# PoseLib/PoseLib

Hardware: AMD Instinct MI355X
Metric: scored RANSAC hypotheses/sec (P3P@5k corrs, 5pt@5k corrs) (higher is better)
Workload: dtype f64; 1 GPU; p3p_5000; correspondences=5000, problems_in_flight_per_gpu=128, distinct_scenes=64

## Files before the change

### poselib_amd/csrc/kernels.hip

```cpp
#include "pl_kernels.h"
#include "pl_global.h"
#include "pl_lm_chain.inc"
#include "pl_device.h"
#include <atomic>
#include "pl_prefilter.h"
#include <cstdlib>
#include "pl_sampler.h"
#include "pl_solver_h4.h"
#include "pl_solver_p3p.h"
#include "pl_solver_p5lp_radial.h"
#include "pl_solver_rel.h"

namespace pl {

typedef const float __attribute__((address_space(4))) *uniform_f32_ptr;
typedef const double __attribute__((address_space(4))) *uniform_f64_ptr;
typedef const uint32_t __attribute__((address_space(4))) *uniform_u32_ptr;
__device__ __forceinline__ uniform_f32_ptr as_uniform(const float *p) { return (uniform_f32_ptr)(uintptr_t)p; }
__device__ __forceinline__ uniform_f64_ptr as_uniform(const double *p) { return (uniform_f64_ptr)(uintptr_t)p; }
__device__ __forceinline__ uniform_u32_ptr as_uniform(const uint32_t *p) { return (uniform_u32_ptr)(uintptr_t)p; }

__device__ __forceinline__ double wave_sum(double v) {
#pragma unroll
    for (int off = 32; off > 0; off >>= 1)
// ... 1084 lines not shown
        }
    };
    __builtin_amdgcn_fence(__ATOMIC_ACQ_REL, "wavefront");
    Batch b0, b1;
    fetch(n0, first, b0);
    if (n1) {
        fetch(n1, first + n0, b1);
        finish(b0);
        finish(b1);
    } else {
        finish(b0);
    }
}

template <int PG>
__device__ __forceinline__ void abs16_tile_bits(const half8_t (&Aop)[kAbs16Dirs], const uint4 (&s_b)[1 + kAbs16Dirs][PG][32], int col, int half,
                                                uint32_t (&out)[16]) {
#pragma unroll
    for (int v = 0; v < 16; ++v)
        out[v] = 0u;
    const float16_t kZero = {0, 0, 0, 0, 0, 0, 0, 0, 0, 0, 0, 0, 0, 0, 0, 0};
    auto products = [&](int g, float16_t &D0, float16_t &D1, float16_t &D2) {
        half8_t Bop[kAbs16Dirs];
#pragma unroll
        for (int d = 0; d < kAbs16Dirs; ++d) {
            const uint4 braw = s_b[half ? 1 + d : 0][g][col];
            __builtin_memcpy(&Bop[d], &braw, 16);
        }
        D0 = __builtin_amdgcn_mfma_f32_32x32x16_f16(Aop[0], Bop[0], kZero, 0, 0, 0);
        D1 = __builtin_amdgcn_mfma_f32_32x32x16_f16(Aop[1], Bop[1], kZero, 0, 0, 0);
        D2 = __builtin_amdgcn_mfma_f32_32x32x16_f16(Aop[2], Bop[2], kZero, 0, 0, 0);
    };
    float16_t D0, D1, D2;
    products(0, D0, D1, D2);
#pragma unroll 16
    for (int g = 1; g < PG; ++g) {
        uint32_t T[16];
#pragma unroll
        for (int v = 0; v < 16; ++v)
            T[v] = __float_as_uint(D0[v]) | __float_as_uint(D1[v]) | __float_as_uint(D2[v]);
        products(g, D0, D1, D2);
#pragma unroll
        for (int v = 0; v < 16; ++v)
            out[v] = __builtin_amdgcn_alignbit(out[v], T[v], 31);
        __builtin_amdgcn_sched_group_barrier(0x002, 16, 0);
        __builtin_amdgcn_sched_group_barrier(0x100, 3, 0);
        __builtin_amdgcn_sched_group_barrier(0x002, 4, 0);
        __builtin_amdgcn_sched_group_barrier(0x008, 1, 0);
        __builtin_amdgcn_sched_group_barrier(0x002, 4, 0);
        __builtin_amdgcn_sched_group_barrier(0x008, 1, 0);
        __builtin_amdgcn_sched_group_barrier(0x002, 4, 0);
        __builtin_amdgcn_sched_group_barrier(0x008, 1, 0);
        __builtin_amdgcn_sched_group_barrier(0x002, 4, 0);
    }
#pragma unroll
    for (int v = 0; v < 16; ++v) {
        const uint32_t sg = __float_as_uint(D0[v]) | __float_as_uint(D1[v]) | __float_as_uint(D2[v]);
        out[v] = __builtin_amdgcn_alignbit(out[v], sg, 31);
    }
}

constexpr int kScoreAll = 0, kScoreLead = 1, kScoreSel = 2, kScoreCount = 3, kScoreCountAll = 4;
template <int PG, int MODE = kScoreAll>
__device__ __forceinline__ void score_mfma_body(const PointSet &pts, const uint4 *__restrict__ shadow16,
                                                const uint4 *__restrict__ points16,
                                                const double *__restrict__ models, const uint32_t *__restrict__ slots,
                                                const uint32_t *__restrict__ num_hyp_ptr, uint32_t hyp_capacity,
                                                double thr2, uint32_t *__restrict__ part_count,
                                                double *__restrict__ part_score, uint32_t slice, uint32_t chunk,
                                                uint32_t nslices, const uint32_t *__restrict__ sel = nullptr,
                                                uint32_t lead = 0) {
    constexpr int kWaves = kMfmaThreads / 64;
    constexpr int NPW = 32 * PG;
    __shared__ double s_pts[5][NPW];
    __shared__ uint16_t s_queue[kWaves][kMfmaQueueCap];
    __shared__ double s_acc_s[kWaves][64];
    __shared__ uint32_t s_acc_c[kWaves][64];
    __shared__ uint32_t s_next_unit;
    __shared__ uint4 s_b[1 + kAbs16Dirs][PG][32];
    const int lane = threadIdx.x & 63;
    const int wave = __builtin_amdgcn_readfirstlane((int)(threadIdx.x >> 6));
    const int col = lane & 31, half = lane >> 5;

    uint32_t validbits = 0;
#pragma unroll
    for (int g = 0; g < PG; ++g)
        validbits |= (chunk * NPW + g * 32 + col < pts.n) ? (1u << (PG - 1 - g)) : 0u;
    const uint4 *const prow = points16 + (size_t)chunk * NPW * 4;
    for (uint32_t j = threadIdx.x; j < (uint32_t)NPW; j += kMfmaThreads) {
        const uint32_t i = chunk * NPW + j;
        const uint32_t ic = i < pts.n ? i : 0u;
#pragma unroll
        for (int d = 0; d < 5; ++d)
            s_pts[d][j] = pts.a[d][ic];
#pragma unroll
        for (int r = 0; r < 1 + kAbs16Dirs; ++r)
            s_b[r][j >> 5][j & 31] = prow[(size_t)j * 4 + r];
    }
    if (threadIdx.x == 0)
        s_next_unit = 0;
    __syncthreads();

    const uint32_t H = MODE == kScoreLead ? min(*as_uniform(num_hyp_ptr), lead) : *as_uniform(num_hyp_ptr);
    uint16_t *const queue = s_queue[wave];
    double *const acc_s = s_acc_s[wave];
    uint32_t *const acc_c = s_acc_c[wave];
    const uint32_t waves_per_chunk = nslices * kWaves;
    auto request_ticket = [&]() -> uint32_t {
        uint32_t t = 0;
        if (lane == 0) {
            const uint32_t k = atomicAdd(&s_next_unit, 1u);
            t = slice * kWaves + (k % kWaves) + (k / kWaves) * waves_per_chunk;
        }
        return t;
    };
    uint32_t ticket = (uint32_t)__builtin_amdgcn_readfirstlane((int)request_ticket());
    uint32_t kb, gn;
    while (unit_of_ticket<32u>(ticket, H, waves_per_chunk, kb, gn)) {
        const uint32_t pending = request_ticket();
        uint32_t unit_pos = 0;
        if constexpr (MODE == kScoreSel)
            unit_pos = sel ? sel[kb + min((uint32_t)lane, gn - 1u)] : kb + min((uint32_t)lane, gn - 1u);
        const uint32_t unit_slots = slots[MODE == kScoreSel ? unit_pos : kb + min((uint32_t)lane, gn - 1u)];
        acc_s[lane] = 0.0;
        acc_c[lane] = 0;
        uint32_t qhead = 0, qtail = 0;

        auto drain_pair = [&](uint32_t n2) {
            mfma_drain<EST_ABS>(queue, qhead, 64u, n2, &s_pts[0][0], NPW, models, unit_slots, thr2, acc_s, acc_c);
            qhead += 64u + n2;
        };
        auto drain = [&](uint32_t n) {
            mfma_drain<EST_ABS>(queue, qhead, n, 0u, &s_pts[0][0], NPW, models, unit_slots, thr2, acc_s, acc_c);
            qhead += n;
        };

        const uint32_t ngroups32 = (gn + 31u) / 32u;
        auto load_a = [&](uint32_t hg, uint4 (&A)[kAbs16Dirs]) {
            const uint4 *row = shadow16 + (size_t)(kb + 32u * hg + (uint32_t)col) * 4;
            if constexpr (MODE == kScoreSel)
                row = shadow16 + (size_t)(uint32_t)__shfl((int)unit_pos, (int)(32u * hg + (uint32_t)col), 64) * 4;
#pragma unroll
            for (int d = 0; d < kAbs16Dirs; ++d)
                A[d] = row[half ? 3 : d];
        };
        uint4 Araw[kAbs16Dirs];
        load_a(0, Araw);
        for (uint32_t hg = 0; hg < ngroups32; ++hg) {
            half8_t Aop[kAbs16Dirs];
#pragma unroll
            for (int d = 0; d < kAbs16Dirs; ++d)
                __builtin_memcpy(&Aop[d], &Araw[d], 16);
            if (hg + 1 < ngroups32)
                load_a(hg + 1, Araw);
            uint32_t out[16];
            abs16_tile_bits<PG>(Aop, s_b, col, half, out);
            const bool partial_group = hg * 32u + 32u > gn;
            auto expand_round = [&](int v, bool check_slot) {
                const uint32_t slot = hg * 32u + 8u * (uint32_t)(v >> 2) + 4u * (uint32_t)half + (uint32_t)(v & 3);
                uint32_t bits = ~out[v] & validbits;
                if (check_slot && slot >= gn)
                    bits = 0u;
                const uint64_t anyb = __builtin_amdgcn_ballot_w64(bits != 0u);
                if (anyb) {
                    const uint32_t cnt = (uint32_t)__popc(bits);
                    if (!__builtin_amdgcn_ballot_w64(cnt > 1u)) {
                        const uint32_t below = __builtin_amdgcn_mbcnt_hi((uint32_t)(anyb >> 32), __builtin_amdgcn_mbcnt_lo((uint32_t)anyb, 0u));
                        if (bits) {
                            const uint32_t g = (uint32_t)(PG - 1 - (31 - __clz((int)bits)));
                            queue[(qtail + below) & (kMfmaQueueCap - 1)] = (uint16_t)((slot << 9) | (g * 32u + (uint32_t)col));
                        }
                        qtail += (uint32_t)__popcll(anyb);
                    } else {
                        const uint32_t incl = wave_scan_u32(cnt);
                        const uint32_t total = (uint32_t)__builtin_amdgcn_readlane((int)incl, 63);
                        uint32_t pos = qtail + incl - cnt;
                        uint32_t rest = bits;
                        while (rest) {
                            const int hi = 31 - __clz((int)rest);
                            rest &= ~(1u << hi);
                            const uint32_t g = (uint32_t)(PG - 1 - hi);
                            queue[pos & (kMfmaQueueCap - 1)] = (uint16_t)((slot << 9) | (g * 32u + (uint32_t)col));
                            ++pos;
                        }
                        qtail += total;
                    }
                    while (qtail - qhead >= 128u)
                        drain_pair(64u);
                }
            };
            if (partial_group) {
#pragma unroll
                for (int v = 0; v < 16; ++v)
                    expand_round(v, true);
            } else {
#pragma unroll
                for (int v = 0; v < 16; ++v)
                    expand_round(v, false);
            }
        }
        if (qtail - qhead > 64u)
            drain_pair(qtail - qhead - 64u);
        else if (qtail != qhead)
            drain(qtail - qhead);
        __builtin_amdgcn_fence(__ATOMIC_ACQ_REL, "wavefront");
        if ((uint32_t)lane < gn) {
            const size_t o = MODE == kScoreSel ? (size_t)chunk * hyp_capacity + unit_pos : (size_t)chunk * hyp_capacity + kb + lane;
            part_score[o] = acc_s[lane];
            part_count[o] = acc_c[lane];
        }
        ticket = (uint32_t)__builtin_amdgcn_readfirstlane((int)pending);
    }
}

template <int PG>
__device__ __forceinline__ void score_count_body(uint32_t n_points, const uint4 *__restrict__ shadow16, const uint4 *__restrict__ points16,
                                                 const uint32_t *__restrict__ num_hyp_ptr, uint32_t hyp_capacity,
                                                 uint32_t *__restrict__ survivors, uint32_t slice, uint32_t chunk, uint32_t nslices,
                                                 uint32_t first) {
    constexpr int kWaves = kMfmaThreads / 64;
    constexpr int NPW = 32 * PG;
    __shared__ uint4 s_b[1 + kAbs16Dirs][PG][32];
    __shared__ uint32_t s_cnt[kWaves][64];
    __shared__ uint32_t s_next_unit;
    const int lane = threadIdx.x & 63;
    const int wave = __builtin_amdgcn_readfirstlane((int)(threadIdx.x >> 6));
    const int col = lane & 31, half = lane >> 5;
    uint32_t validbits = 0;
#pragma unroll
    for (int g = 0; g < PG; ++g)
        validbits |= (chunk * NPW + g * 32 + col < n_points) ? (1u << (PG - 1 - g)) : 0u;
    const uint4 *const prow = points16 + (size_t)chunk * NPW * 4;
    for (uint32_t j = threadIdx.x; j < (uint32_t)NPW; j += kMfmaThreads) {
#pragma unroll
        for (int r = 0; r < 1 + kAbs16Dirs; ++r)
            s_b[r][j >> 5][j & 31] = prow[(size_t)j * 4 + r];
    }
    if (threadIdx.x == 0)
        s_next_unit = 0;
    __syncthreads();

    const uint32_t Hall = *as_uniform(num_hyp_ptr);
    if (Hall <= first)
        return;
    const uint32_t H = Hall - first;
    uint32_t *const cnt = s_cnt[wave];
    const uint32_t waves_per_chunk = nslices * kWaves;
    auto request_ticket = [&]() -> uint32_t {
        uint32_t t = 0;
        if (lane == 0) {
            const uint32_t k = atomicAdd(&s_next_unit, 1u);
            t = slice * kWaves + (k % kWaves) + (k / kWaves) * waves_per_chunk;
        }
        return t;
    };
    uint32_t ticket = (uint32_t)__builtin_amdgcn_readfirstlane((int)request_ticket());
    uint32_t kb, gn;
    while (unit_of_ticket<32u>(ticket, H, waves_per_chunk, kb, gn)) {
        const uint32_t pending = request_ticket();
        const uint32_t ngroups32 = (gn + 31u) / 32u;
        auto load_a = [&](uint32_t hg, uint4 (&A)[kAbs16Dirs]) {
            const uint4 *row = shadow16 + (size_t)min(first + kb + 32u * hg + (uint32_t)col, Hall - 1u) * 4;
#pragma unroll
            for (int d = 0; d < kAbs16Dirs; ++d)
                A[d] = row[half ? 3 : d];
        };
        uint4 Araw[kAbs16Dirs];
        load_a(0, Araw);
        for (uint32_t hg = 0; hg < ngroups32; ++hg) {
            half8_t Aop[kAbs16Dirs];
#pragma unroll
            for (int d = 0; d < kAbs16Dirs; ++d)
                __builtin_memcpy(&Aop[d], &Araw[d], 16);
            if (hg + 1 < ngroups32)
                load_a(hg + 1, Araw);
            uint32_t out[16];
            abs16_tile_bits<PG>(Aop, s_b, col, half, out);
            uint32_t pk[6] = {0u, 0u, 0u, 0u, 0u, 0u};
#pragma unroll
            for (int v = 0; v < 16; ++v)
                pk[v / 3] += (uint32_t)__popc(~out[v] & validbits) << (10 * (v % 3));
#pragma unroll
            for (int j = 0; j < 6; ++j) {
                uint32_t s = pk[j];
                s += dpp_shift_u32<0x111>(s);
                s += dpp_shift_u32<0x112>(s);
                s += dpp_shift_u32<0x114>(s);
                s += dpp_shift_u32<0x118>(s);
                s += dpp_shift_u32<0x142, 0xa>(s);
                pk[j] = s;
            }
            if (col == 31) {
#pragma unroll
                for (int v = 0; v < 16; ++v)
                    cnt[hg * 32u + 8u * (uint32_t)(v >> 2) + 4u * (uint32_t)half + (uint32_t)(v & 3)] = (pk[v / 3] >> (10 * (v % 3))) & 0x3ffu;
            }
        }
        __builtin_amdgcn_fence(__ATOMIC_ACQ_REL, "wavefront");
        if ((uint32_t)lane < gn)
            survivors[(size_t)chunk * hyp_capacity + first + kb + lane] = cnt[lane];
        __builtin_amdgcn_fence(__ATOMIC_ACQ_REL, "wavefront");
        ticket = (uint32_t)__builtin_amdgcn_readfirstlane((int)pending);
    }
}

template <int PG>
__global__ __launch_bounds__(kMfmaThreads) __attribute__((amdgpu_waves_per_eu(4, 8))) void k_score_mfma(PointSet pts, const uint4 *__restrict__ shadow16,
                                                               const uint4 *__restrict__ points16,
                                                               const double *__restrict__ models,
                                                               const uint32_t *__restrict__ slots,
                                                               const uint32_t *__restrict__ num_hyp_ptr,
                                                               uint32_t hyp_capacity, double thr2,
                                                               uint32_t *__restrict__ part_count,
                                                               double *__restrict__ part_score,
                                                               uint32_t *__restrict__ tickets) {
    (void)tickets;
    uint32_t slice, chunk;
    slice_chunk_of_workgroup(gridDim.x, gridDim.y, slice, chunk);
    score_mfma_body<PG>(pts, shadow16, points16, models, slots, num_hyp_ptr, hyp_capacity, thr2, part_count, part_score, slice,
                        chunk, gridDim.x);
}
template <int PG>
__global__ __launch_bounds__(kMfmaThreads) __attribute__((amdgpu_waves_per_eu(4, 8))) void k_score_mfma_g(const GroupArgs *ga) {
    const GroupArgs &g = ga[blockIdx.z];
    uint32_t slice, chunk;
    if (!g.active || !g.use_mfma || !slice_chunk_of_workgroup(g.slices, g.chunks, slice, chunk))
        return;
    const ScoreArgs a = globalised(g.score);
    score_mfma_body<PG>(a.pts, static_cast<const uint4 *>(a.shadow16), static_cast<const uint4 *>(a.points16), a.models, a.slots,
                        a.num_hyp, a.hyp_capacity, a.thr2, a.part_count, a.part_score, slice, chunk, g.slices);
// ... 104 lines not shown
    uint32_t cs = 0;
    for (uint32_t ch = 0; ch < cstar; ++ch)
        cs += a.part_count[(size_t)ch * a.hyp_capacity + p];
    return prune_rule(cs, 0.0, S, N, a.thr2, *pr.st) ? 0u : 1u;
}
__global__ __launch_bounds__(256) void k_prune_label(ScoreArgs a) {
    const PruneArgs &pr = a.prune;
    const uint32_t H = *a.num_hyp, cstar = pr.st->cstar, p = blockIdx.x * 256u + threadIdx.x;
    if (p >= H || p < pr.lead || cstar >= pr.chunks || pr.kept[p] != kKept)
        return;
    const uint32_t N = a.pts.n, S = min(cstar * pr.chunk_points, N);
    uint32_t cs = 0;
    double sum = 0.0;
    for (uint32_t ch = 0; ch < cstar; ++ch) {
        cs += a.part_count[(size_t)ch * a.hyp_capacity + p];
        sum += a.part_score[(size_t)ch * a.hyp_capacity + p];
    }
    if (prune_rule(cs, sum, S, N, a.thr2, *pr.st))
        pr.kept[p] = kPrunedExact;
}
__device__ __forceinline__ void prune_flags_body(const ScoreArgs &a) {
    __shared__ uint32_t wt[16];
    const PruneArgs &pr = a.prune;
    const uint32_t H = *a.num_hyp, cstar = pr.st->cstar;
    if (blockIdx.x * 1024u >= H)
        return;
    const uint32_t p = blockIdx.x * 1024u + threadIdx.x;
    const uint32_t keep = prune_keeps(a, p, H, cstar);
    if (p < H)
        pr.kept[p] = (uint8_t)keep;
    const uint32_t tot = wave_sum_u32(keep);
    if ((threadIdx.x & 63) == 0)
        wt[threadIdx.x >> 6] = tot;
    __syncthreads();
    if (threadIdx.x == 0) {
        uint32_t t = 0;
        for (int w = 0; w < 16; ++w)
            t += wt[w];
        pr.blk_kept[blockIdx.x] = t;
    }
}
__device__ __forceinline__ void prune_list_body(const ScoreArgs &a) {
    __shared__ uint32_t wt[16], wb[16];
    const PruneArgs &pr = a.prune;
    const uint32_t H = *a.num_hyp;
    if (blockIdx.x * 1024u >= H)
        return;
    const int lane = threadIdx.x & 63, wave = threadIdx.x >> 6;
    uint32_t before = 0;
    for (uint32_t j = threadIdx.x; j < blockIdx.x; j += 1024u)
        before += pr.blk_kept[j];
    before = wave_sum_u32(before);
    const uint32_t p = blockIdx.x * 1024u + threadIdx.x;
    const uint32_t keep = p < H ? (uint32_t)pr.kept[p] : 0u;
    const uint32_t inc = wave_scan_u32(keep);
    if (lane == 63)
        wt[wave] = inc;
    if (lane == 0)
        wb[wave] = before;
    __syncthreads();
    uint32_t at = inc - keep;
    for (int w = 0; w < 16; ++w)
        at += wb[w] + (w < wave ? wt[w] : 0u);
    if (keep)
        pr.sel[at] = p;
    if (p == H - 1u)
        pr.st->sel_len = at + keep;
}
__global__ __launch_bounds__(1024) void k_prune_flags(ScoreArgs a) { prune_flags_body(a); }
__global__ __launch_bounds__(1024) void k_prune_list(ScoreArgs a) { prune_list_body(a); }
__global__ __launch_bounds__(1024) void k_prune_flags_g(const GroupArgs *ga) {
    const GroupArgs &g = ga[blockIdx.z];
    if (!g.active || !g.use_mfma || !g.score.prune.st)
        return;
    prune_flags_body(globalised(g.score));
}
__global__ __launch_bounds__(1024) void k_prune_list_g(const GroupArgs *ga) {
    const GroupArgs &g = ga[blockIdx.z];
    if (!g.active || !g.use_mfma || !g.score.prune.st)
        return;
    prune_list_body(globalised(g.score));
}

constexpr int kBoundThreads = 256;
template <int P, bool RESID>
__device__ __forceinline__ void score_bound_body(const ScoreArgs &a, uint32_t slice, uint32_t chunk, uint32_t nslices) {
    constexpr int kWaves = kBoundThreads / 64;
    constexpr uint32_t NPW = 64u * P;
    const PruneArgs &pr = a.prune;
    if (!pr.st || !pr.bound || *as_uniform(&pr.st->cstar) >= pr.chunks)
        return;
    const uint32_t first = RESID ? 0u : min(*as_uniform(a.num_hyp), pr.lead), len = *as_uniform(&pr.st->sel_len);
    if (len <= first)
        return;
    const int lane = threadIdx.x & 63;
    const int wave = __builtin_amdgcn_readfirstlane((int)(threadIdx.x >> 6));
    const PrefilterArgs pf = a.pf;
    float x[P], y[P], X[P], Y[P], Z[P], fw[P];
    bool valid[P];
    uint64_t vmask[P];
#pragma unroll
    for (int p = 0; p < P; ++p) {
        const uint32_t i = chunk * NPW + (uint32_t)p * 64u + (uint32_t)lane;
        valid[p] = i < a.pts.n;
        vmask[p] = __builtin_amdgcn_ballot_w64(valid[p]);
        const uint32_t ic = valid[p] ? i : 0u;
        const double Xd = a.pts.a[2][ic], Yd = a.pts.a[3][ic], Zd = a.pts.a[4][ic];
        x[p] = (float)a.pts.a[0][ic], y[p] = (float)a.pts.a[1][ic];
        X[p] = (float)Xd, Y[p] = (float)Yd, Z[p] = (float)Zd;
        fw[p] = pf_point_abs(Xd, Yd, Zd, pf.gx);
    }
    const uint32_t nent = len - first;
    for (uint32_t u = slice * kWaves + (uint32_t)wave; u * 64u < nent; u += nslices * kWaves) {
        const uint32_t e = first + u * 64u + (uint32_t)lane;
        const uint32_t pos = pr.sel[min(e, len - 1u)];
        const float4 *sh = reinterpret_cast<const float4 *>(a.models + (size_t)a.slots[pos] * kModelStride + kShadowOff);
        float4 rv[4];
#pragma unroll
        for (int k = 0; k < 4; ++k)
            rv[k] = sh[k];
        const uint32_t n = min(64u, nent - u * 64u);
        uint32_t my_c = 0, my_q = 0;
        for (uint32_t j = 0; j < n; ++j) {
            float r[16];
#pragma unroll
            for (int k = 0; k < 4; ++k) {
                r[4 * k + 0] = __builtin_bit_cast(float, __builtin_amdgcn_readlane(__builtin_bit_cast(int, rv[k].x), (int)j));
                r[4 * k + 1] = __builtin_bit_cast(float, __builtin_amdgcn_readlane(__builtin_bit_cast(int, rv[k].y), (int)j));
                r[4 * k + 2] = __builtin_bit_cast(float, __builtin_amdgcn_readlane(__builtin_bit_cast(int, rv[k].z), (int)j));
                r[4 * k + 3] = __builtin_bit_cast(float, __builtin_amdgcn_readlane(__builtin_bit_cast(int, rv[k].w), (int)j));
            }
            const float gt = pf_abs_bound_slack(r, pf.gx);
            uint32_t c = 0, q = 0;
            if constexpr (RESID) {
#pragma unroll
                for (int p = 0; p < P; ++p) {
                    const float L = pf_abs_r2_lower(r, gt, x[p], y[p], X[p], Y[p], Z[p], fw[p]);
                    c += (uint32_t)__popcll(__builtin_amdgcn_ballot_w64(valid[p] && L < pf.thr2_up));
                    q += valid[p] ? pf_bound_quantum(L, pf.inv_thr2_dn) : 0u;
                }
                q = (uint32_t)__builtin_amdgcn_readlane((int)wave_scan_u32(q), 63);
            } else {
#pragma unroll
                for (int p = 0; p + 1 < P; p += 2) {
                    const v2f Xp = {X[p], X[p + 1]}, Yp = {Y[p], Y[p + 1]}, Zp = {Z[p], Z[p + 1]};
                    const v2f xp = {x[p], x[p + 1]}, yp = {y[p], y[p + 1]}, w = {fw[p], fw[p + 1]};
                    const v2f z0 = pk_fma(bc(r[0]), Xp, pk_fma(bc(r[1]), Yp, pk_fma(bc(r[2]), Zp, bc(r[9]))));
                    const v2f z1 = pk_fma(bc(r[3]), Xp, pk_fma(bc(r[4]), Yp, pk_fma(bc(r[5]), Zp, bc(r[10]))));
                    const v2f z2 = pk_fma(bc(r[6]), Xp, pk_fma(bc(r[7]), Yp, pk_fma(bc(r[8]), Zp, bc(r[11]))));
                    const v2f a0 = pk_fma(-xp, z2, z0);
                    const v2f a1 = pk_fma(-yp, z2, z1);
                    const v2f W = w + bc(gt);
                    const v2f B = pk_fma(bc(pf.thr), z2, W);
#pragma unroll
                    for (int e2 = 0; e2 < 2; ++e2) {
                        const uint64_t out = vmask[p + e2] & (__builtin_amdgcn_ballot_w64(fmaxf(fabsf(a0[e2]), fabsf(a1[e2])) > B[e2]) |
                                                              __builtin_amdgcn_ballot_w64(z2[e2] < -W[e2]));
                        q += (uint32_t)__popcll(out);
                        c += (uint32_t)__popcll(vmask[p + e2] & ~out);
                    }
                }
                if constexpr (P & 1) {
                    constexpr int p = P - 1;
                    const uint64_t out = vmask[p] & __builtin_amdgcn_ballot_w64(pf_abs_outlier(r, gt, pf.thr, x[p], y[p], X[p], Y[p], Z[p], fw[p]));
                    q += (uint32_t)__popcll(out);
                    c += (uint32_t)__popcll(vmask[p] & ~out);
                }
                q <<= 20;
            }
            if ((uint32_t)lane == j)
                my_c = c, my_q = q;
        }
        if ((uint32_t)lane < n) {
            const size_t o = (size_t)chunk * a.hyp_capacity + pos;
            a.part_count[o] = my_c;
            a.part_score[o] = (double)my_q;
        }
    }
}
template <int P, bool RESID> __global__ __launch_bounds__(kBoundThreads) void k_score_bound(ScoreArgs a) {
    uint32_t slice, chunk;
    slice_chunk_of_workgroup(gridDim.x, gridDim.y, slice, chunk);
    score_bound_body<P, RESID>(a, slice, chunk, gridDim.x);
}
template <bool RESID> __global__ __launch_bounds__(kBoundThreads) void k_score_bound_g(const GroupArgs *ga) {
    const GroupArgs &g = ga[blockIdx.z];
    uint32_t slice, chunk;
    const uint32_t ns = pruned_slices<kScoreSel>(g.slices);
    if (!g.active || !g.use_mfma || !g.score.prune.st || !slice_chunk_of_workgroup(ns, g.chunks, slice, chunk))
        return;
    score_bound_body<5, RESID>(globalised(g.score), slice, chunk, ns);
}
__device__ __forceinline__ void prune_bound_body(const ScoreArgs &a, int stage) {
    __shared__ uint32_t wt[16];
    const PruneArgs &pr = a.prune;
    if (!pr.bound || pr.st->cstar >= pr.chunks)
        return;
    const uint32_t first = stage ? 0u : min(*a.num_hyp, pr.lead), len = pr.st->sel_len;
    const uint32_t lead_max = pr.st->lead_max;
    const double beat = pr.st->lead_min * (1.0 + kPruneScoreMargin);
    const int lane = threadIdx.x & 63, wave = threadIdx.x >> 6;
    uint32_t base = 0;
    __syncthreads();
    for (uint32_t t0 = first; t0 < len; t0 += 1024u) {
        const uint32_t e = t0 + threadIdx.x;
        uint32_t keep = 0, p = 0;
        if (e < len) {
            p = pr.sel[e];
            uint32_t c = 0;
            uint64_t q = 0;
#pragma unroll 8
            for (uint32_t ch = 0; ch < pr.chunks; ++ch) {
                c += a.part_count[(size_t)ch * a.hyp_capacity + p];
                q += (uint64_t)a.part_score[(size_t)ch * a.hyp_capacity + p];
            }
            const double qd = (double)q * 9.5367431640625e-07;
            double s_lb = a.thr2 * qd;
            if (fma(a.thr2, qd, -s_lb) < 0.0)
                s_lb = __longlong_as_double(__double_as_longlong(s_lb) - 1);
            keep = (c <= lead_max && s_lb > beat) ? 0u : 1u;
            if (!keep)
                pr.kept[p] = kDropped;
            if (pr.bnd_count)
                pr.bnd_count[p] = c, pr.bnd_score[p] = s_lb;
        }
        const uint32_t inc = wave_scan_u32(keep);
        if (lane == 63)
            wt[wave] = inc;
        __syncthreads();
        uint32_t at = base + inc - keep, tot = 0;
        for (int w = 0; w < 16; ++w) {
            at += w < wave ? wt[w] : 0u;
            tot += wt[w];
        }
        if (keep)
            pr.sel[at] = p;
        base += tot;
        __syncthreads();
    }
    if (threadIdx.x == 0)
        pr.st->sel_len = base;
}
__global__ __launch_bounds__(1024) void k_prune_bound(ScoreArgs a, int stage) { prune_bound_body(a, stage); }
__global__ __launch_bounds__(1024) void k_prune_bound_g(const GroupArgs *ga, int stage) {
    const GroupArgs &g = ga[blockIdx.z];
    if (!g.active || !g.use_mfma || !g.score.prune.st)
        return;
    prune_bound_body(globalised(g.score), stage);
}



template <int EST, int PG>
__device__ __forceinline__ void score_mfma2_body(const PointSet &pts, const uint4 *__restrict__ hypop,
                                                 const double *__restrict__ models, const uint32_t *__restrict__ slots,
                                                 const uint32_t *__restrict__ num_hyp_ptr, uint32_t hyp_capacity,
                                                 double thr2, const PrefilterArgs &pf, uint32_t *__restrict__ part_count,
                                                 double *__restrict__ part_score, uint32_t slice, uint32_t chunk,
                                                 uint32_t nslices) {
    static_assert(EST == EST_REL || EST == EST_FUND, "Sampson scores");
    constexpr int kWaves = kMfmaThreads / 64;
    constexpr int NPW = 32 * PG;
    constexpr int NBR = (EST == EST_REL) ? 6 : 1;
    __shared__ double s_pts[4][NPW];
    __shared__ double s_bear[NBR][(EST == EST_REL) ? NPW : 1];
    __shared__ uint16_t s_queue[kWaves][kMfmaQueueCap];
    __shared__ double s_acc_s[kWaves][64];
    __shared__ uint32_t s_acc_c[kWaves][64];
    __shared__ uint32_t s_next_unit;
    __shared__ uint4 s_bop[PG][3][64];
    const int lane = threadIdx.x & 63;
    const int wave = __builtin_amdgcn_readfirstlane((int)(threadIdx.x >> 6));
    const int col = lane & 31, half = lane >> 5;

    for (uint32_t j = threadIdx.x; j < (uint32_t)NPW; j += kMfmaThreads) {
        const uint32_t i = chunk * NPW + j;
        const uint32_t ic = i < pts.n ? i : 0u;
        const double a0 = pts.a[0][ic], a1 = pts.a[1][ic], b0 = pts.a[2][ic], b1 = pts.a[3][ic];
        s_pts[0][j] = a0, s_pts[1][j] = a1, s_pts[2][j] = b0, s_pts[3][j] = b1;
        if constexpr (EST == EST_REL) {
            const Vec3 u1 = bearing(a0, a1), u2 = bearing(b0, b1);
            s_bear[0][j] = u1.x, s_bear[1][j] = u1.y, s_bear[2][j] = u1.z;
            s_bear[3][j] = u2.x, s_bear[4][j] = u2.y, s_bear[5][j] = u2.z;
        }
    }
    uint32_t validbits = 0;
#pragma unroll
    for (int g = 0; g < PG; ++g)
        validbits |= (chunk * NPW + g * 32 + col < pts.n) ? (1u << (PG - 1 - g)) : 0u;
    for (uint32_t j = threadIdx.x; j < (uint32_t)NPW; j += kMfmaThreads) {
        const uint32_t i = chunk * NPW + j;
        const bool valid = i < pts.n;
        const uint32_t ic = valid ? i : 0u;
        Sampson16Operand o;
        pf16_sampson_point(pts.a[0][ic], pts.a[1][ic], pts.a[2][ic], pts.a[3][ic], valid, pf.t16, o);
#pragma unroll
        for (int b = 0; b < 6; ++b) {
            const uint16_t *h = b < 4 ? o.c + 8 * b : o.s + 8 * (b - 4);
            s_bop[j >> 5][b >> 1][(j & 31) + 32 * (b & 1)] =
                make_uint4((uint32_t)h[0] | ((uint32_t)h[1] << 16), (uint32_t)h[2] | ((uint32_t)h[3] << 16),
                           (uint32_t)h[4] | ((uint32_t)h[5] << 16), (uint32_t)h[6] | ((uint32_t)h[7] << 16));
        }
    }
    if (threadIdx.x == 0)
        s_next_unit = 0;
    __syncthreads();

    const uint32_t H = *as_uniform(num_hyp_ptr);
    const float t16 = pf.t16;
    uint16_t *const queue = s_queue[wave];
    double *const acc_s = s_acc_s[wave];
    uint32_t *const acc_c = s_acc_c[wave];
    const uint32_t waves_per_chunk = nslices * kWaves;
    auto request_ticket = [&]() -> uint32_t {
        uint32_t t = 0;
        if (lane == 0) {
            const uint32_t k = atomicAdd(&s_next_unit, 1u);
            t = slice * kWaves + (k % kWaves) + (k / kWaves) * waves_per_chunk;
        }
        return t;
    };
    uint32_t ticket = (uint32_t)__builtin_amdgcn_readfirstlane((int)request_ticket());
    uint32_t kb, gn;
    while (unit_of_ticket(ticket, H, waves_per_chunk, kb, gn)) {
        const uint32_t pending = request_ticket();
        const uint32_t unit_slots = slots[kb + min((uint32_t)lane, gn - 1u)];
        acc_s[lane] = 0.0;
        acc_c[lane] = 0;
        uint32_t qhead = 0, qtail = 0;

        auto drain = [&](uint32_t n) {
// ... 1934 lines not shown
        k_score_mfma<2 * PP><<<mgrid, mblock, 0, stream>>>(a.pts, static_cast<const uint4 *>(a.shadow16),                \
                                                         static_cast<const uint4 *>(a.points16), a.models, a.slots,    \
                                                         a.num_hyp, a.hyp_capacity, a.thr2, a.part_count, a.part_score, \
                                                         a.tickets);                                                   \
        break;
            switch (P) {
                PL_M_CASE(1)
                PL_M_CASE(2)
                PL_M_CASE(3)
                PL_M_CASE(4)
                PL_M_CASE(5)
            default:
                return hipErrorInvalidValue;
            }
#undef PL_M_CASE
            return hipGetLastError();
        }
    }
    if (streaming) {
        const dim3 qgrid(std::max<uint32_t>(1u, slices * (uint32_t)kScoreThreads / (uint32_t)kQueueThreads), chunks);
        const dim3 qblock(kQueueThreads);
#define PL_Q_CASE(PP)                                                                                                  \
    case PP:                                                                                                           \
        k_score_queue<E, PP><<<qgrid, qblock, 0, stream>>>(a.pts, a.shadow, a.compact64, a.num_hyp, a.hyp_capacity,      \
                                                         a.thr2, pf, a.part_count, a.part_score, a.tickets);           \
        break;
        switch (P) {
            PL_Q_CASE(1)
            PL_Q_CASE(2)
            PL_Q_CASE(3)
            PL_Q_CASE(4)
            PL_Q_CASE(5)
            PL_Q_CASE(6)
        default:
            return hipErrorInvalidValue;
        }
#undef PL_Q_CASE
        return hipGetLastError();
    }
    return hipErrorInvalidValue;
}

hipError_t launch_score_seq(int est, const SeqScoreArgs &a, hipStream_t stream) {
    if (a.cap == 0)
        return hipSuccess;
    const dim3 grid(std::min<uint32_t>(a.cap, 128u)), block(kSeqThreads);
    PL_DISPATCH_EST_0TO5(est, k_score_seq<E><<<grid, block, 0, stream>>>(a));
    return hipGetLastError();
}
int tangent_score_chunk() { return kTangentChunk; }
int radial1d_score_chunk() { return kRadialChunk; }
hipError_t launch_prune_lead(const ScoreArgs &a, hipStream_t stream) {
    k_prune_lead<<<dim3(1), dim3(256), 0, stream>>>(a);
    return hipGetLastError();
}
hipError_t launch_prune_select(const ScoreArgs &a, hipStream_t stream) {
    const uint32_t nb = std::max<uint32_t>(1u, (a.hyp_capacity + 1023u) / 1024u);
    k_prune_flags<<<dim3(nb), dim3(1024), 0, stream>>>(a);
    k_prune_list<<<dim3(nb), dim3(1024), 0, stream>>>(a);
    return hipGetLastError();
}
hipError_t launch_group_prune_lead(const GroupArgs *args, const GroupDims &d, hipStream_t stream) {
    k_prune_lead_g<<<dim3(1, 1, d.G), dim3(256), 0, stream>>>(args);
    return hipGetLastError();
}
hipError_t launch_group_prune_select(const GroupArgs *args, const GroupDims &d, hipStream_t stream) {
    const uint32_t nb = std::max<uint32_t>(1u, (d.max_hcap + 1023u) / 1024u);
    k_prune_flags_g<<<dim3(nb, 1, d.G), dim3(1024), 0, stream>>>(args);
    k_prune_list_g<<<dim3(nb, 1, d.G), dim3(1024), 0, stream>>>(args);
    return hipGetLastError();
}
template <int PG> static hipError_t launch_score_pruned_pg(const ScoreArgs &a, dim3 grid, hipStream_t stream) {
    const dim3 block(kMfmaThreads);
    const dim3 lead_grid(pruned_slices<kScoreLead>(grid.x), grid.y), sel_grid(pruned_slices<kScoreSel>(grid.x), grid.y);
    k_score_mfma_pr<PG, kScoreLead><<<lead_grid, block, 0, stream>>>(a);
    hipError_t e = launch_prune_lead(a, stream);
    if (e != hipSuccess)
        return e;
    k_score_mfma_pr<PG, kScoreCount><<<grid, block, 0, stream>>>(a);
    e = launch_prune_select(a, stream);
    if (e != hipSuccess)
        return e;
    if (a.prune.bound) {
        k_score_bound<PG / 2, false><<<sel_grid, dim3(kBoundThreads), 0, stream>>>(a);
        k_prune_bound<<<dim3(1), dim3(1024), 0, stream>>>(a, 0);
        k_score_bound<PG / 2, true><<<sel_grid, dim3(kBoundThreads), 0, stream>>>(a);
        k_prune_bound<<<dim3(1), dim3(1024), 0, stream>>>(a, 1);
    }
    k_score_mfma_pr<PG, kScoreSel><<<sel_grid, block, 0, stream>>>(a);
    return hipGetLastError();
}
static hipError_t pruned_grid(const ScoreArgs &a, uint32_t slices, dim3 &grid, int &P) {
    uint32_t chunks;
    score_shape(EST_ABS, a.pts.n, true, true, chunks, P);
    if (!a.shadow16 || !a.points16 || !a.prune.st || a.prune.chunks != chunks || a.prune.chunk_points != 64u * (uint32_t)P)
        return hipErrorInvalidValue;
    const uint32_t mslices = std::min<uint32_t>(slices * (uint32_t)kScoreThreads / (uint32_t)kMfmaThreads,
                                                score_slice_limit(EST_ABS, chunks, true));
    grid = dim3(xcd_slices(mslices), chunks);
    return (P == 4 || P == 5) ? hipSuccess : hipErrorInvalidValue;
}
hipError_t launch_score_pruned(const ScoreArgs &a, uint32_t slices, hipStream_t stream) {
    dim3 grid;
    int P;
    const hipError_t e = pruned_grid(a, slices, grid, P);
    if (e != hipSuccess)
        return e;
    return P == 4 ? launch_score_pruned_pg<8>(a, grid, stream) : launch_score_pruned_pg<10>(a, grid, stream);
}
hipError_t launch_score_count(const ScoreArgs &a, uint32_t slices, hipStream_t stream) {
    dim3 grid;
    int P;
    const hipError_t e = pruned_grid(a, slices, grid, P);
    if (e != hipSuccess)
        return e;
    if (P == 4)
        k_score_mfma_pr<8, kScoreCountAll><<<grid, dim3(kMfmaThreads), 0, stream>>>(a);
    else
        k_score_mfma_pr<10, kScoreCountAll><<<grid, dim3(kMfmaThreads), 0, stream>>>(a);
    return hipGetLastError();
}
hipError_t launch_prune_label(const ScoreArgs &a, hipStream_t stream) {
    k_prune_label<<<dim3(std::max<uint32_t>(1u, (a.hyp_capacity + 255u) / 256u)), dim3(256), 0, stream>>>(a);
    return hipGetLastError();
}

hipError_t launch_score(int est, const ScoreArgs &a, uint32_t slices, hipStream_t stream) {
    if (est == EST_RAD1D) {
        if (!a.shadow || !a.compact64)
            return hipErrorInvalidValue;
        const uint32_t chunks = score_chunks(est, a.pts.n, true, false);
        const dim3 qgrid(std::max<uint32_t>(1u, slices * (uint32_t)kScoreThreads / (uint32_t)kQueueThreads), chunks);
        k_score_radial1d<<<qgrid, dim3(kQueueThreads), 0, stream>>>(a.pts, a.shadow, a.compact64, a.num_hyp, a.hyp_capacity, a.thr2, a.pf,
                                                                    a.part_count, a.part_score);
        return hipGetLastError();
    }
    if (est == EST_RELT) {
        if (!a.shadow || !a.compact64)
            return hipErrorInvalidValue;
        const uint32_t chunks = score_chunks(est, a.pts.n, true, false);
        const dim3 qgrid(std::max<uint32_t>(1u, slices * (uint32_t)kScoreThreads / (uint32_t)kQueueThreads), chunks);
        k_score_tangent<<<qgrid, dim3(kQueueThreads), 0, stream>>>(a.pts, a.shadow, a.compact64, a.num_hyp, a.hyp_capacity, a.thr2, a.pf,
                                                                   a.part_count, a.part_score);
        return hipGetLastError();
    }
    PL_DISPATCH_EST(est, return launch_score_est<E>(a, slices, stream));
    return hipSuccess;
}


hipError_t launch_lm(int est, const PointSet &pts, LMTask *tasks, uint32_t num_tasks, hipStream_t stream) {
    const size_t want = sizeof(double) * point_doubles(est) * (size_t)pts.n;
    return launch_lm_tasks(est, tasks, num_tasks, want <= 128 * 1024 ? pts.n : 0u, stream);
}
static std::atomic<int> g_lm_mode{-1};
void set_lm_mode(int mode) { g_lm_mode.store((mode == 1 || mode == 2) ? mode : 0, std::memory_order_release); }
int get_lm_mode() {
    int m = g_lm_mode.load(std::memory_order_acquire);
    if (m < 0) {
        const char *e = std::getenv("POSELIB_AMD_LM_ORDERED");
        m = (e && e[0] == '1') ? 1 : (e && e[0] == '2') ? 2 : 0;
        g_lm_mode.store(m, std::memory_order_release);
    }
    return m;
}
static thread_local int tl_lm_force_ordered = 0;
void set_lm_force_ordered(int on) { tl_lm_force_ordered = on; }
bool lm_sums_ordered(int est) {
    if (tl_lm_force_ordered)
        return true;
// ... 51 lines not shown
        PL_DISPATCH_EST_0123_5(est, k_lm_ordered<E><<<dim3(num_tasks), dim3(kLMThreads), bytes, stream>>>(tasks, (uint32_t)bytes));
    } else {
        PL_DISPATCH_EST_0TO5(est, k_lm<E><<<dim3(num_tasks), dim3(kLMThreads), bytes, stream>>>(tasks, (uint32_t)bytes));
    }
    return hipGetLastError();
}

__global__ void k_task_records(int est, const LMTask *tasks, const double *records_in, double *records_out,
                               uint32_t num_tasks, LMTask *host_tasks) {
    const uint32_t j = blockIdx.x * blockDim.x + threadIdx.x;
    if (j >= num_tasks)
        return;
    if (host_tasks) {
        for (int i = 0; i < kParamDoubles; ++i)
            host_tasks[j].params[i] = tasks[j].params[i];
        host_tasks[j].iterations = tasks[j].iterations;
        host_tasks[j].skipped = tasks[j].skipped;
        host_tasks[j].cost = tasks[j].cost;
        host_tasks[j].initial_cost = tasks[j].initial_cost;
    }
    double *out = records_out + (size_t)j * kModelStride;
    if (tasks[j].skipped) {
        for (int i = 0; i < kModelStride; ++i)
            out[i] = records_in[(size_t)j * kModelStride + i];
    } else {
        record_from_lm_params(est, tasks[j].params, out);
    }
}
__global__ void k_select_record(const double *score_refined, double incumbent_score, const double *rec_refined,
                                const double *rec_incumbent, double *out) {
    const double *src = (*score_refined < incumbent_score) ? rec_refined : rec_incumbent;
    if (threadIdx.x < kModelStride)
        out[threadIdx.x] = src[threadIdx.x];
}
__global__ void k_select_record_g(const SelectArgs *arr) {
    const SelectArgs a = globalised(arr[blockIdx.z]);
    if (!a.out)
        return;
    const double *src = (*a.score_refined < a.incumbent_score) ? a.rec_refined : a.rec_incumbent;
    if (threadIdx.x < kModelStride)
        a.out[threadIdx.x] = src[threadIdx.x];
    if (threadIdx.x == 63 && a.fetch_src)
        *a.fetch_dst = *a.fetch_src;
    if (threadIdx.x == 62 && a.count_out)
        *a.count_out = (*a.score_refined < a.incumbent_score) ? *a.count_refined : a.count_incumbent;
}
hipError_t launch_group_select(const SelectArgs *args, uint32_t G, hipStream_t stream) {
    if (G == 0)
        return hipSuccess;
    k_select_record_g<<<dim3(1, 1, G), dim3(64), 0, stream>>>(args);
    return hipGetLastError();
}
hipError_t launch_group_mask(int est, const MaskArgs *args, uint32_t G, uint32_t max_n, hipStream_t stream) {
    if (G == 0 || max_n == 0)
        return hipSuccess;
    const dim3 grid((max_n + 255) / 256, 1, G), block(256);
    PL_DISPATCH_EST(est, k_mask_g<E><<<grid, block, 0, stream>>>(args));
    return hipGetLastError();
}
hipError_t launch_group_score_seq(int est, const SeqScoreArgs *args, uint32_t G, uint32_t max_cap, hipStream_t stream) {
    if (G == 0 || max_cap == 0)
        return hipSuccess;
    const dim3 grid(std::min<uint32_t>(max_cap, 128u), 1, G), block(kSeqThreads);
    PL_DISPATCH_EST(est, k_score_seq_g<E><<<grid, block, 0, stream>>>(args));
    return hipGetLastError();
}

int group_points_per_lane(int est) { return (est == EST_REL || est == EST_FUND) ? 6 : 5; }

template <int E> static hipError_t launch_group_score_est(const GroupArgs *args, const GroupDims &d, hipStream_t stream) {
    const dim3 grid(std::max<uint32_t>(1u, d.max_slices), std::max<uint32_t>(1u, d.max_chunks), d.G);
    if constexpr (E == EST_ABS) {
        if (d.any_mfma && d.any_prune) {
            const dim3 lead_grid(pruned_slices<kScoreLead>(grid.x), grid.y, grid.z), sel_grid(pruned_slices<kScoreSel>(grid.x), grid.y, grid.z);
            k_score_mfma_pr_g<10, kScoreLead><<<lead_grid, dim3(kMfmaThreads), 0, stream>>>(args);
            hipError_t e = launch_group_prune_lead(args, d, stream);
            if (e != hipSuccess)
                return e;
            k_score_mfma_pr_g<10, kScoreCount><<<grid, dim3(kMfmaThreads), 0, stream>>>(args);
            e = launch_group_prune_select(args, d, stream);
            if (e != hipSuccess)
                return e;
            if (d.any_bound) {
                k_score_bound_g<false><<<sel_grid, dim3(kBoundThreads), 0, stream>>>(args);
                k_prune_bound_g<<<dim3(1, 1, d.G), dim3(1024), 0, stream>>>(args, 0);
                k_score_bound_g<true><<<sel_grid, dim3(kBoundThreads), 0, stream>>>(args);
                k_prune_bound_g<<<dim3(1, 1, d.G), dim3(1024), 0, stream>>>(args, 1);
            }
            k_score_mfma_pr_g<10, kScoreSel><<<sel_grid, dim3(kMfmaThreads), 0, stream>>>(args);
        } else if (d.any_mfma)
            k_score_mfma_g<10><<<grid, dim3(kMfmaThreads), 0, stream>>>(args);
        if (d.any_queue)
            k_score_queue_g<EST_ABS, 5><<<grid, dim3(kQueueThreads), 0, stream>>>(args);
    } else if constexpr (E == EST_HOM) {
        if (d.any_mfma)
            k_score_mfmah_g<10><<<grid, dim3(kMfmaThreads), 0, stream>>>(args);
        if (d.any_queue)
            k_score_queue_g<EST_HOM, 5><<<grid, dim3(kQueueThreads), 0, stream>>>(args);
    } else {
        if (d.any_mfma)
            k_score_mfma2_g<E, 2 * group_mfma2_points_per_lane(E)><<<grid, dim3(kMfmaThreads), 0, stream>>>(args);
        if (d.any_queue)
            k_score_queue_g<E, 6><<<grid, dim3(kQueueThreads), 0, stream>>>(args);
    }
    return hipGetLastError();
}

hipError_t launch_group_score_count(const GroupArgs *args, const GroupDims &d, hipStream_t stream) {
    const dim3 grid(std::max<uint32_t>(1u, d.max_slices), std::max<uint32_t>(1u, d.max_chunks), d.G);
    k_score_mfma_pr_g<10, kScoreCountAll><<<grid, dim3(kMfmaThreads), 0, stream>>>(args);
    return hipGetLastError();
}
hipError_t launch_group_score(int est, const GroupArgs *args, const GroupDims &d, hipStream_t stream) {
    if (d.G == 0)
        return hipSuccess;
    hipError_t e = hipSuccess;
    PL_DISPATCH_EST(est, e = launch_group_score_est<E>(args, d, stream));
    return e;
}

hipError_t launch_group_generate(int est, const GroupArgs *args, uint32_t max_B, uint32_t G, hipStream_t stream) {
    if (G == 0 || max_B == 0)
        return hipSuccess;
    if (est == EST_REL)
        return launch_group_generate_rel(args, max_B, G, stream);
    const dim3 ggrid((max_B + 63) / 64, 1, G), gblock(64);
    PL_DISPATCH_EST(est, k_generate_g<E><<<ggrid, gblock, 0, stream>>>(args));
    return hipGetLastError();
}

hipError_t launch_group_batch(int est, const GroupArgs *args, const GroupDims &d, hipStream_t stream, hipEvent_t ev0,
                              hipEvent_t ev1) {
    if (d.G == 0)
        return hipSuccess;
    hipError_t e = launch_group_positions(sample_size(est), args, d, stream);
    if (e != hipSuccess)
        return e;
    e = launch_group_generate(est, args, d.max_B, d.G, stream);
    if (e != hipSuccess)
        return e;
    e = launch_group_compact(args, d, stream);
    if (e != hipSuccess)
        return e;
    if (ev0 && (e = hipEventRecord(ev0, stream)) != hipSuccess)
        return e;
    e = launch_group_score(est, args, d, stream);
    if (e != hipSuccess)
        return e;
    if (ev1 && (e = hipEventRecord(ev1, stream)) != hipSuccess)
        return e;
    e = launch_group_finalize_records(args, d, stream);
    if (e != hipSuccess)
        return e;
    const uint32_t per_problem = std::max<uint32_t>(16u, std::min<uint32_t>(128u, 4096u / std::max<uint32_t>(1u, d.G)));
    const dim3 sgrid(per_problem, 1, d.G), sblock(kSeqThreads);
    PL_DISPATCH_EST(est, k_score_seq_gb<E><<<sgrid, sblock, 0, stream>>>(args));
    return hipGetLastError();
}

hipError_t launch_task_records(int est, const LMTask *tasks, const double *records_in, double *records_out,
                               uint32_t num_tasks, LMTask *host_tasks, hipStream_t stream) {
    if (num_tasks == 0)
        return hipSuccess;
    k_task_records<<<dim3((num_tasks + 63) / 64), dim3(64), 0, stream>>>(est, tasks, records_in, records_out, num_tasks,
                                                                         host_tasks);
    return hipGetLastError();
}
hipError_t launch_select_record(const double *score_refined, double incumbent_score, const double *rec_refined,
                                const double *rec_incumbent, double *out, hipStream_t stream) {
    k_select_record<<<dim3(1), dim3(64), 0, stream>>>(score_refined, incumbent_score, rec_refined, rec_incumbent, out);
// ... 40 lines not shown
```

Before: 1.268 billion hypotheses/s.

## Fuse two-stage bound scoring into one kernel with in-block reduction and early exit

Merges the cheap bound pass, its prune, the residual bound pass and the second prune into a single k_score_bound kernel. It runs on a fixed grid of 16 workgroups of 512 threads, with waves striding over chunks and per-hypothesis partial counts reduced in shared memory instead of global part_count/part_score arrays. Only hypotheses that survive the first bound are rescored with the residual bound, and the final prune kernel just compacts the list. It also adds an early return in the MFMA score bodies for workgroups with no ticket, done before the shared-memory loads. In exchange, the fixed small grid and non-resident chunk reloads may limit parallelism when there are many hypotheses or chunks.

```diff
diff --git a/poselib_amd/csrc/kernels.hip b/poselib_amd/csrc/kernels.hip
--- a/poselib_amd/csrc/kernels.hip
+++ b/poselib_amd/csrc/kernels.hip
@@ -1190,6 +1190,14 @@
     const int wave = __builtin_amdgcn_readfirstlane((int)(threadIdx.x >> 6));
     const int col = lane & 31, half = lane >> 5;
 
+    const uint32_t H = MODE == kScoreLead ? min(*as_uniform(num_hyp_ptr), lead) : *as_uniform(num_hyp_ptr);
+    const uint32_t waves_per_chunk = nslices * kWaves;
+    {
+        uint32_t kb0, gn0;
+        if (!unit_of_ticket<32u>(slice * kWaves, H, waves_per_chunk, kb0, gn0))
+            return;
+    }
+
     uint32_t validbits = 0;
 #pragma unroll
     for (int g = 0; g < PG; ++g)
@@ -1209,11 +1217,9 @@
         s_next_unit = 0;
     __syncthreads();
 
-    const uint32_t H = MODE == kScoreLead ? min(*as_uniform(num_hyp_ptr), lead) : *as_uniform(num_hyp_ptr);
     uint16_t *const queue = s_queue[wave];
     double *const acc_s = s_acc_s[wave];
     uint32_t *const acc_c = s_acc_c[wave];
-    const uint32_t waves_per_chunk = nslices * kWaves;
     auto request_ticket = [&]() -> uint32_t {
         uint32_t t = 0;
         if (lane == 0) {
@@ -1334,6 +1340,16 @@
     const int lane = threadIdx.x & 63;
     const int wave = __builtin_amdgcn_readfirstlane((int)(threadIdx.x >> 6));
     const int col = lane & 31, half = lane >> 5;
+    const uint32_t Hall = *as_uniform(num_hyp_ptr);
+    if (Hall <= first)
+        return;
+    const uint32_t H = Hall - first;
+    const uint32_t waves_per_chunk = nslices * kWaves;
+    {
+        uint32_t kb0, gn0;
+        if (!unit_of_ticket<32u>(slice * kWaves, H, waves_per_chunk, kb0, gn0))
+            return;
+    }
     uint32_t validbits = 0;
 #pragma unroll
     for (int g = 0; g < PG; ++g)
@@ -1348,12 +1364,7 @@
         s_next_unit = 0;
     __syncthreads();
 
-    const uint32_t Hall = *as_uniform(num_hyp_ptr);
-    if (Hall <= first)
-        return;
-    const uint32_t H = Hall - first;
     uint32_t *const cnt = s_cnt[wave];
-    const uint32_t waves_per_chunk = nslices * kWaves;
     auto request_ticket = [&]() -> uint32_t {
         uint32_t t = 0;
         if (lane == 0) {
@@ -1624,36 +1635,66 @@
     prune_list_body(globalised(g.score));
 }
 
-constexpr int kBoundThreads = 256;
-template <int P, bool RESID>
-__device__ __forceinline__ void score_bound_body(const ScoreArgs &a, uint32_t slice, uint32_t chunk, uint32_t nslices) {
+constexpr int kBoundThreads = 512;
+constexpr uint32_t kBoundGroups = 16;
+template <int P> __device__ __forceinline__ void score_bound_body(const ScoreArgs &a, uint32_t wg, uint32_t nwg) {
     constexpr int kWaves = kBoundThreads / 64;
     constexpr uint32_t NPW = 64u * P;
+    __shared__ uint32_t s_c[kWaves][64];
+    __shared__ uint64_t s_q[kWaves][64];
+    __shared__ uint32_t s_und[64];
+    __shared__ uint32_t s_nund;
     const PruneArgs &pr = a.prune;
     if (!pr.st || !pr.bound || *as_uniform(&pr.st->cstar) >= pr.chunks)
         return;
-    const uint32_t first = RESID ? 0u : min(*as_uniform(a.num_hyp), pr.lead), len = *as_uniform(&pr.st->sel_len);
-    if (len <= first)
+    const uint32_t first = min(*as_uniform(a.num_hyp), pr.lead), len = *as_uniform(&pr.st->sel_len);
+    if (len <= first || (uint64_t)wg * 64u >= len - first)
         return;
     const int lane = threadIdx.x & 63;
     const int wave = __builtin_amdgcn_readfirstlane((int)(threadIdx.x >> 6));
     const PrefilterArgs pf = a.pf;
+    const uint32_t chunks = pr.chunks;
+    const bool resident = chunks <= (uint32_t)kWaves;
     float x[P], y[P], X[P], Y[P], Z[P], fw[P];
     bool valid[P];
     uint64_t vmask[P];
-#pragma unroll
-    for (int p = 0; p < P; ++p) {
-        const uint32_t i = chunk * NPW + (uint32_t)p * 64u + (uint32_t)lane;
-        valid[p] = i < a.pts.n;
-        vmask[p] = __builtin_amdgcn_ballot_w64(valid[p]);
-        const uint32_t ic = valid[p] ? i : 0u;
-        const double Xd = a.pts.a[2][ic], Yd = a.pts.a[3][ic], Zd = a.pts.a[4][ic];
-        x[p] = (float)a.pts.a[0][ic], y[p] = (float)a.pts.a[1][ic];
-        X[p] = (float)Xd, Y[p] = (float)Yd, Z[p] = (float)Zd;
-        fw[p] = pf_point_abs(Xd, Yd, Zd, pf.gx);
-    }
+    auto load_chunk = [&](uint32_t chunk) {
+#pragma unroll
+        for (int p = 0; p < P; ++p) {
+            const uint32_t i = chunk * NPW + (uint32_t)p * 64u + (uint32_t)lane;
+            valid[p] = i < a.pts.n;
+            vmask[p] = __builtin_amdgcn_ballot_w64(valid[p]);
+            const uint32_t ic = valid[p] ? i : 0u;
+            const double Xd = a.pts.a[2][ic], Yd = a.pts.a[3][ic], Zd = a.pts.a[4][ic];
+            x[p] = (float)a.pts.a[0][ic], y[p] = (float)a.pts.a[1][ic];
+            X[p] = (float)Xd, Y[p] = (float)Yd, Z[p] = (float)Zd;
+            fw[p] = pf_point_abs(Xd, Yd, Zd, pf.gx);
+        }
+    };
+    load_chunk(min((uint32_t)wave, chunks - 1u));
+    const uint32_t lead_max = pr.st->lead_max;
+    const double beat = pr.st->lead_min * (1.0 + kPruneScoreMargin);
+    auto decide = [&](uint32_t pos) -> bool {
+        uint32_t c = 0;
+        uint64_t q = 0;
+#pragma unroll
+        for (int w = 0; w < kWaves; ++w) {
+            c += s_c[w][lane];
+            q += s_q[w][lane];
+        }
+        const double qd = (double)q * 9.5367431640625e-07;
+        double s_lb = a.thr2 * qd;
+        if (fma(a.thr2, qd, -s_lb) < 0.0)
+            s_lb = __longlong_as_double(__double_as_longlong(s_lb) - 1);
+        const bool keep = !(c <= lead_max && s_lb > beat);
+        if (!keep)
+            pr.kept[pos] = kDropped;
+        if (pr.bnd_count)
+            pr.bnd_count[pos] = c, pr.bnd_score[pos] = s_lb;
+        return keep;
+    };
     const uint32_t nent = len - first;
-    for (uint32_t u = slice * kWaves + (uint32_t)wave; u * 64u < nent; u += nslices * kWaves) {
+    for (uint32_t u = wg; (uint64_t)u * 64u < nent; u += nwg) {
         const uint32_t e = first + u * 64u + (uint32_t)lane;
         const uint32_t pos = pr.sel[min(e, len - 1u)];
         const float4 *sh = reinterpret_cast<const float4 *>(a.models + (size_t)a.slots[pos] * kModelStride + kShadowOff);
@@ -1662,9 +1703,7 @@
         for (int k = 0; k < 4; ++k)
             rv[k] = sh[k];
         const uint32_t n = min(64u, nent - u * 64u);
-        uint32_t my_c = 0, my_q = 0;
-        for (uint32_t j = 0; j < n; ++j) {
-            float r[16];
+        auto model_of_lane = [&](uint32_t j, float (&r)[16]) {
 #pragma unroll
             for (int k = 0; k < 4; ++k) {
                 r[4 * k + 0] = __builtin_bit_cast(float, __builtin_amdgcn_readlane(__builtin_bit_cast(int, rv[k].x), (int)j));
@@ -1672,17 +1711,17 @@
                 r[4 * k + 2] = __builtin_bit_cast(float, __builtin_amdgcn_readlane(__builtin_bit_cast(int, rv[k].z), (int)j));
                 r[4 * k + 3] = __builtin_bit_cast(float, __builtin_amdgcn_readlane(__builtin_bit_cast(int, rv[k].w), (int)j));
             }
-            const float gt = pf_abs_bound_slack(r, pf.gx);
-            uint32_t c = 0, q = 0;
-            if constexpr (RESID) {
-#pragma unroll
-                for (int p = 0; p < P; ++p) {
-                    const float L = pf_abs_r2_lower(r, gt, x[p], y[p], X[p], Y[p], Z[p], fw[p]);
-                    c += (uint32_t)__popcll(__builtin_amdgcn_ballot_w64(valid[p] && L < pf.thr2_up));
-                    q += valid[p] ? pf_bound_quantum(L, pf.inv_thr2_dn) : 0u;
-                }
-                q = (uint32_t)__builtin_amdgcn_readlane((int)wave_scan_u32(q), 63);
-            } else {
+        };
+        uint32_t my_c = 0;
+        uint64_t my_q = 0;
+        for (uint32_t ch = (uint32_t)wave; ch < chunks; ch += (uint32_t)kWaves) {
+            if (!resident)
+                load_chunk(ch);
+            for (uint32_t j = 0; j < n; ++j) {
+                float r[16];
+                model_of_lane(j, r);
+                const float gt = pf_abs_bound_slack(r, pf.gx);
+                uint32_t c = 0, q = 0;
 #pragma unroll
                 for (int p = 0; p + 1 < P; p += 2) {
                     const v2f Xp = {X[p], X[p + 1]}, Yp = {Y[p], Y[p + 1]}, Zp = {Z[p], Z[p + 1]};
@@ -1708,39 +1747,68 @@
                     q += (uint32_t)__popcll(out);
                     c += (uint32_t)__popcll(vmask[p] & ~out);
                 }
-                q <<= 20;
-            }
-            if ((uint32_t)lane == j)
-                my_c = c, my_q = q;
-        }
-        if ((uint32_t)lane < n) {
-            const size_t o = (size_t)chunk * a.hyp_capacity + pos;
-            a.part_count[o] = my_c;
-            a.part_score[o] = (double)my_q;
-        }
-    }
-}
-template <int P, bool RESID> __global__ __launch_bounds__(kBoundThreads) void k_score_bound(ScoreArgs a) {
-    uint32_t slice, chunk;
-    slice_chunk_of_workgroup(gridDim.x, gridDim.y, slice, chunk);
-    score_bound_body<P, RESID>(a, slice, chunk, gridDim.x);
-}
-template <bool RESID> __global__ __launch_bounds__(kBoundThreads) void k_score_bound_g(const GroupArgs *ga) {
+                if ((uint32_t)lane == j)
+                    my_c += c, my_q += q;
+            }
+        }
+        s_c[wave][lane] = my_c;
+        s_q[wave][lane] = my_q << 20;
+        __syncthreads();
+        bool open = false;
+        if (wave == 0) {
+            open = (uint32_t)lane < n && decide(pos);
+            const uint64_t und = __builtin_amdgcn_ballot_w64(open);
+            if (open)
+                s_und[__builtin_amdgcn_mbcnt_hi((uint32_t)(und >> 32), __builtin_amdgcn_mbcnt_lo((uint32_t)und, 0u))] = (uint32_t)lane;
+            if (lane == 0)
+                s_nund = (uint32_t)__popcll(und);
+        }
+        __syncthreads();
+        const uint32_t nund = (uint32_t)__builtin_amdgcn_readfirstlane((int)s_nund);
+        if (nund) {
+            my_c = 0, my_q = 0;
+            for (uint32_t ch = (uint32_t)wave; ch < chunks; ch += (uint32_t)kWaves) {
+                if (!resident)
+                    load_chunk(ch);
+                for (uint32_t k = 0; k < nund; ++k) {
+                    const uint32_t j = (uint32_t)__builtin_amdgcn_readfirstlane((int)s_und[k]);
+                    float r[16];
+                    model_of_lane(j, r);
+                    const float gt = pf_abs_bound_slack(r, pf.gx);
+                    uint32_t c = 0, q = 0;
+#pragma unroll
+                    for (int p = 0; p < P; ++p) {
+                        const float L = pf_abs_r2_lower(r, gt, x[p], y[p], X[p], Y[p], Z[p], fw[p]);
+                        c += (uint32_t)__popcll(__builtin_amdgcn_ballot_w64(valid[p] && L < pf.thr2_up));
+                        q += valid[p] ? pf_bound_quantum(L, pf.inv_thr2_dn) : 0u;
+                    }
+                    q = (uint32_t)__builtin_amdgcn_readlane((int)wave_scan_u32(q), 63);
+                    if ((uint32_t)lane == j)
+                        my_c += c, my_q += q;
+                }
+            }
+            s_c[wave][lane] = my_c;
+            s_q[wave][lane] = my_q;
+            __syncthreads();
+            if (open)
+                (void)decide(pos);
+        }
+        __syncthreads();
+    }
+}
+template <int P> __global__ __launch_bounds__(kBoundThreads) void k_score_bound(ScoreArgs a) { score_bound_body<P>(a, blockIdx.x, gridDim.x); }
+__global__ __launch_bounds__(kBoundThreads) void k_score_bound_g(const GroupArgs *ga) {
     const GroupArgs &g = ga[blockIdx.z];
-    uint32_t slice, chunk;
-    const uint32_t ns = pruned_slices<kScoreSel>(g.slices);
-    if (!g.active || !g.use_mfma || !g.score.prune.st || !slice_chunk_of_workgroup(ns, g.chunks, slice, chunk))
+    if (!g.active || !g.use_mfma || !g.score.prune.st)
         return;
-    score_bound_body<5, RESID>(globalised(g.score), slice, chunk, ns);
-}
-__device__ __forceinline__ void prune_bound_body(const ScoreArgs &a, int stage) {
+    score_bound_body<5>(globalised(g.score), blockIdx.x, gridDim.x);
+}
+__device__ __forceinline__ void prune_bound_body(const ScoreArgs &a) {
     __shared__ uint32_t wt[16];
     const PruneArgs &pr = a.prune;
     if (!pr.bound || pr.st->cstar >= pr.chunks)
         return;
-    const uint32_t first = stage ? 0u : min(*a.num_hyp, pr.lead), len = pr.st->sel_len;
-    const uint32_t lead_max = pr.st->lead_max;
-    const double beat = pr.st->lead_min * (1.0 + kPruneScoreMargin);
+    const uint32_t first = min(*a.num_hyp, pr.lead), len = pr.st->sel_len;
     const int lane = threadIdx.x & 63, wave = threadIdx.x >> 6;
     uint32_t base = 0;
     __syncthreads();
@@ -1749,22 +1817,7 @@
         uint32_t keep = 0, p = 0;
         if (e < len) {
             p = pr.sel[e];
-            uint32_t c = 0;
-            uint64_t q = 0;
-#pragma unroll 8
-            for (uint32_t ch = 0; ch < pr.chunks; ++ch) {
-                c += a.part_count[(size_t)ch * a.hyp_capacity + p];
-                q += (uint64_t)a.part_score[(size_t)ch * a.hyp_capacity + p];
-            }
-            const double qd = (double)q * 9.5367431640625e-07;
-            double s_lb = a.thr2 * qd;
-            if (fma(a.thr2, qd, -s_lb) < 0.0)
-                s_lb = __longlong_as_double(__double_as_longlong(s_lb) - 1);
-            keep = (c <= lead_max && s_lb > beat) ? 0u : 1u;
-            if (!keep)
-                pr.kept[p] = kDropped;
-            if (pr.bnd_count)
-                pr.bnd_count[p] = c, pr.bnd_score[p] = s_lb;
+            keep = pr.kept[p] != kDropped ? 1u : 0u;
         }
         const uint32_t inc = wave_scan_u32(keep);
         if (lane == 63)
@@ -1783,12 +1836,12 @@
     if (threadIdx.x == 0)
         pr.st->sel_len = base;
 }
-__global__ __launch_bounds__(1024) void k_prune_bound(ScoreArgs a, int stage) { prune_bound_body(a, stage); }
-__global__ __launch_bounds__(1024) void k_prune_bound_g(const GroupArgs *ga, int stage) {
+__global__ __launch_bounds__(1024) void k_prune_bound(ScoreArgs a) { prune_bound_body(a); }
+__global__ __launch_bounds__(1024) void k_prune_bound_g(const GroupArgs *ga) {
     const GroupArgs &g = ga[blockIdx.z];
     if (!g.active || !g.use_mfma || !g.score.prune.st)
         return;
-    prune_bound_body(globalised(g.score), stage);
+    prune_bound_body(globalised(g.score));
 }
 
 
@@ -3889,10 +3942,8 @@
     if (e != hipSuccess)
         return e;
     if (a.prune.bound) {
-        k_score_bound<PG / 2, false><<<sel_grid, dim3(kBoundThreads), 0, stream>>>(a);
-        k_prune_bound<<<dim3(1), dim3(1024), 0, stream>>>(a, 0);
-        k_score_bound<PG / 2, true><<<sel_grid, dim3(kBoundThreads), 0, stream>>>(a);
-        k_prune_bound<<<dim3(1), dim3(1024), 0, stream>>>(a, 1);
+        k_score_bound<PG / 2><<<dim3(kBoundGroups), dim3(kBoundThreads), 0, stream>>>(a);
+        k_prune_bound<<<dim3(1), dim3(1024), 0, stream>>>(a);
     }
     k_score_mfma_pr<PG, kScoreSel><<<sel_grid, block, 0, stream>>>(a);
     return hipGetLastError();
@@ -4110,10 +4161,8 @@
             if (e != hipSuccess)
                 return e;
             if (d.any_bound) {
-                k_score_bound_g<false><<<sel_grid, dim3(kBoundThreads), 0, stream>>>(args);
-                k_prune_bound_g<<<dim3(1, 1, d.G), dim3(1024), 0, stream>>>(args, 0);
-                k_score_bound_g<true><<<sel_grid, dim3(kBoundThreads), 0, stream>>>(args);
-                k_prune_bound_g<<<dim3(1, 1, d.G), dim3(1024), 0, stream>>>(args, 1);
+                k_score_bound_g<<<dim3(kBoundGroups, 1, d.G), dim3(kBoundThreads), 0, stream>>>(args);
+                k_prune_bound_g<<<dim3(1, 1, d.G), dim3(1024), 0, stream>>>(args);
             }
             k_score_mfma_pr_g<10, kScoreSel><<<sel_grid, dim3(kMfmaThreads), 0, stream>>>(args);
         } else if (d.any_mfma)
```

Measured after the change: 1.300 billion hypotheses/s (median of 6 runs). 2.5% higher.
